# RuyiLian/CheckerPose

Hardware: NVIDIA B200
Metric: RoIs/sec (4096-kpt GNN head) (higher is better)
Workload: dtype bf16

## Files before the change

checkerpose_b200/csrc/sm100.cuh:

```cuda
#pragma once
#include <cuda_runtime.h>
#include <stdint.h>

namespace sm100 {

__device__ __forceinline__ uint32_t smem_u32(const void* p) { return (uint32_t)__cvta_generic_to_shared(p); }

__device__ __forceinline__ void mbar_init(uint64_t* bar, uint32_t count) {
  asm volatile("mbarrier.init.shared::cta.b64 [%0], %1;" ::"r"(smem_u32(bar)), "r"(count) : "memory");
}
__device__ __forceinline__ void fence_mbar_init() { asm volatile("fence.mbarrier_init.release.cluster;" ::: "memory"); }
__device__ __forceinline__ void mbar_arrive_expect_tx(uint64_t* bar, uint32_t bytes) {
  asm volatile("mbarrier.arrive.expect_tx.shared::cta.b64 _, [%0], %1;" ::"r"(smem_u32(bar)), "r"(bytes) : "memory");
}
__device__ __forceinline__ bool mbar_try_wait(uint64_t* bar, uint32_t parity) {
  uint32_t ok;
  asm volatile(
      "{\n\t.reg .pred p;\n\t"
      "mbarrier.try_wait.parity.shared::cta.b64 p, [%1], %2;\n\t"
      "selp.u32 %0, 1, 0, p;\n\t}"
      : "=r"(ok)
      : "r"(smem_u32(bar)), "r"(parity)
      : "memory");
  return ok != 0;
}
__device__ __forceinline__ void mbar_wait(uint64_t* bar, uint32_t parity) {
  if (mbar_try_wait(bar, parity)) return;
  uint32_t spins = 0;
  while (!mbar_try_wait(bar, parity)) {
    if (++spins > (1u << 27)) __trap();
  }
}

__device__ __forceinline__ bool elect_one() {
  uint32_t pred;
  asm volatile(
      "{\n\t.reg .pred p;\n\t"
      "elect.sync _|p, 0xffffffff;\n\t"
      "selp.u32 %0, 1, 0, p;\n\t}"
      : "=r"(pred));
  return pred != 0;
}

__device__ __forceinline__ void fence_proxy_async_smem() { asm volatile("fence.proxy.async.shared::cta;" ::: "memory"); }
__device__ __forceinline__ void tc_fence_before_sync() { asm volatile("tcgen05.fence::before_thread_sync;" ::: "memory"); }
__device__ __forceinline__ void tc_fence_after_sync() { asm volatile("tcgen05.fence::after_thread_sync;" ::: "memory"); }

__device__ __forceinline__ void bulk_g2s(void* smem_dst, const void* gmem_src, uint32_t bytes, uint64_t* bar) {
  asm volatile("cp.async.bulk.shared::cluster.global.mbarrier::complete_tx::bytes [%0], [%1], %2, [%3];" ::"r"(
                   smem_u32(smem_dst)),
               "l"(gmem_src), "r"(bytes), "r"(smem_u32(bar))
               : "memory");
}

__device__ __forceinline__ void tmem_alloc(uint32_t* slot_in_smem, uint32_t ncols) {
  asm volatile("tcgen05.alloc.cta_group::1.sync.aligned.shared::cta.b32 [%0], %1;" ::"r"(smem_u32(slot_in_smem)), "r"(ncols)
               : "memory");
  asm volatile("tcgen05.relinquish_alloc_permit.cta_group::1.sync.aligned;" ::: "memory");
}
__device__ __forceinline__ void tmem_dealloc(uint32_t taddr, uint32_t ncols) {
  asm volatile("tcgen05.dealloc.cta_group::1.sync.aligned.b32 %0, %1;" ::"r"(taddr), "r"(ncols) : "memory");
}

__device__ __forceinline__ void tmem_ld16(uint32_t taddr, uint32_t (&r)[16]) {
  asm volatile(
      "tcgen05.ld.sync.aligned.32x32b.x16.b32 {%0,%1,%2,%3,%4,%5,%6,%7,%8,%9,%10,%11,%12,%13,%14,%15}, [%16];"
      : "=r"(r[0]), "=r"(r[1]), "=r"(r[2]), "=r"(r[3]), "=r"(r[4]), "=r"(r[5]), "=r"(r[6]), "=r"(r[7]), "=r"(r[8]),
        "=r"(r[9]), "=r"(r[10]), "=r"(r[11]), "=r"(r[12]), "=r"(r[13]), "=r"(r[14]), "=r"(r[15])
      : "r"(taddr));
}
__device__ __forceinline__ void tmem_ld_wait() { asm volatile("tcgen05.wait::ld.sync.aligned;" ::: "memory"); }

__device__ __forceinline__ uint64_t make_smem_desc_sw128(uint32_t smem_addr) {
  return (uint64_t)((smem_addr >> 4) & 0x3FFF) | (1ull << 16) | (64ull << 32) | (1ull << 46) | (2ull << 61);
}
__device__ __forceinline__ uint32_t make_idesc_bf16_m128(uint32_t n) {
  return (1u << 4) | (1u << 7) | (1u << 10) | ((n >> 3) << 17) | ((128u >> 4) << 24);
}
__device__ __forceinline__ void mma_bf16_ss(uint32_t d_tmem, uint64_t a_desc, uint64_t b_desc, uint32_t idesc,
                                            uint32_t accumulate) {
  asm volatile(
      "{\n\t.reg .pred p;\n\t"
      "setp.ne.b32 p, %4, 0;\n\t"
      "tcgen05.mma.cta_group::1.kind::f16 [%0], %1, %2, %3, p;\n\t}"
      ::"r"(d_tmem), "l"(a_desc), "l"(b_desc), "r"(idesc), "r"(accumulate)
      : "memory");
}
__device__ __forceinline__ uint32_t smem_desc_lo(uint32_t smem_addr) { return ((smem_addr >> 4) & 0x3FFFu) | (1u << 16); }
__device__ __forceinline__ void mma_bf16_ss_lo(uint32_t d_tmem, uint32_t a_lo, uint32_t b_lo, uint32_t idesc, uint32_t accumulate) {
  asm volatile(
      "{\n\t.reg .pred p;\n\t.reg .b64 da, db;\n\t"
      "setp.ne.b32 p, %4, 0;\n\t"
      "mov.b64 da, {%1, %5};\n\t"
      "mov.b64 db, {%2, %5};\n\t"
      "tcgen05.mma.cta_group::1.kind::f16 [%0], da, db, %3, p;\n\t}"
      ::"r"(d_tmem), "r"(a_lo), "r"(b_lo), "r"(idesc), "r"(accumulate), "r"(0x40004040u)
      : "memory");
}
__device__ __forceinline__ uint32_t cluster_ctarank() {
  uint32_t r;
  asm volatile("mov.u32 %0, %%cluster_ctarank;" : "=r"(r));
  return r;
}
__device__ __forceinline__ void cluster_sync_all() {
  asm volatile("barrier.cluster.arrive.release.aligned;\n\tbarrier.cluster.wait.acquire.aligned;" ::: "memory");
}
__device__ __forceinline__ uint32_t mapa_rank(uint32_t smem_addr, uint32_t rank) {
  uint32_t r;
  asm volatile("mapa.shared::cluster.u32 %0, %1, %2;" : "=r"(r) : "r"(smem_addr), "r"(rank));
  return r;
}
__device__ __forceinline__ void mbar_arrive_cluster(uint32_t cluster_addr) {
  asm volatile("mbarrier.arrive.release.cluster.shared::cluster.b64 _, [%0];" ::"r"(cluster_addr) : "memory");
}
__device__ __forceinline__ void mbar_arrive_remote(uint32_t cluster_addr) {
  asm volatile("mbarrier.arrive.shared::cluster.b64 _, [%0];" ::"r"(cluster_addr) : "memory");
}
__device__ __forceinline__ void tmem_alloc_pair(uint32_t* slot_in_smem, uint32_t ncols) {
  asm volatile("tcgen05.alloc.cta_group::2.sync.aligned.shared::cta.b32 [%0], %1;" ::"r"(smem_u32(slot_in_smem)), "r"(ncols) : "memory");
  asm volatile("tcgen05.relinquish_alloc_permit.cta_group::2.sync.aligned;" ::: "memory");
}
__device__ __forceinline__ void tmem_dealloc_pair(uint32_t taddr, uint32_t ncols) {
  asm volatile("tcgen05.dealloc.cta_group::2.sync.aligned.b32 %0, %1;" ::"r"(taddr), "r"(ncols) : "memory");
}
__device__ __forceinline__ uint32_t make_idesc_bf16(uint32_t m, uint32_t n) {
  return (1u << 4) | (1u << 7) | (1u << 10) | ((n >> 3) << 17) | ((m >> 4) << 24);
}
__device__ __forceinline__ void mma2_bf16_ss_lo(uint32_t d_tmem, uint32_t a_lo, uint32_t b_lo, uint32_t idesc, uint32_t accumulate) {
  asm volatile(
      "{\n\t.reg .pred p;\n\t.reg .b64 da, db;\n\t"
      "setp.ne.b32 p, %4, 0;\n\t"
      "mov.b64 da, {%1, %5};\n\t"
      "mov.b64 db, {%2, %5};\n\t"
      "tcgen05.mma.cta_group::2.kind::f16 [%0], da, db, %3, p;\n\t}"
      ::"r"(d_tmem), "r"(a_lo), "r"(b_lo), "r"(idesc), "r"(accumulate), "r"(0x40004040u)
      : "memory");
}
__device__ __forceinline__ void mma2_commit_both(uint32_t bar_s) {
  asm volatile("tcgen05.commit.cta_group::2.mbarrier::arrive::one.shared::cluster.multicast::cluster.b64 [%0], %1;"
               ::"r"(bar_s), "h"((uint16_t)3) : "memory");
}

__device__ __forceinline__ void bulk_g2s_multicast(void* smem_dst, const void* gmem_src, uint32_t bytes, uint64_t* bar, uint16_t cta_mask) {
  asm volatile("cp.async.bulk.shared::cluster.global.mbarrier::complete_tx::bytes.multicast::cluster [%0], [%1], %2, [%3], %4;"
               ::"r"(smem_u32(smem_dst)), "l"(gmem_src), "r"(bytes), "r"(smem_u32(bar)), "h"(cta_mask) : "memory");
}
__device__ __forceinline__ void mma_commit_multicast(uint64_t* bar, uint16_t cta_mask) {
  asm volatile("tcgen05.commit.cta_group::1.mbarrier::arrive::one.shared::cluster.multicast::cluster.b64 [%0], %1;"
               ::"r"(smem_u32(bar)), "h"(cta_mask) : "memory");
}

__device__ __forceinline__ void mma_commit(uint64_t* bar) {
  asm volatile("tcgen05.commit.cta_group::1.mbarrier::arrive::one.shared::cluster.b64 [%0];" ::"r"(smem_u32(bar))
               : "memory");
}

}
```

checkerpose_b200/csrc/taps_chain_tcgen05.cu:

```cuda
#include <cuda.h>

#include "common.cuh"
#include "sm100.cuh"

using bf16 = __nv_bfloat16;
using namespace sm100;

namespace {

constexpr int TILE_M = 128;
constexpr int NUM_G_WARPS = 4, G_THREADS = NUM_G_WARPS * 32;
constexpr int NUM_E_WARPS = 8;
constexpr int E_WARP0 = 4;
constexpr int W_WARP = E_WARP0 + NUM_E_WARPS, MMA_WARP = W_WARP + 1;
constexpr int NUM_WARPS = 16;
static_assert(NUM_E_WARPS % 4 == 0 && E_WARP0 % 4 == 0 && NUM_G_WARPS <= E_WARP0 && TILE_M % (NUM_G_WARPS * 4) == 0, "epilogue warp w drains TMEM lane quarter w % 4");
constexpr int NTHREADS = NUM_WARPS * 32;
constexpr int CHUNK_BYTES = TILE_M * 128;
constexpr int NX = 4;
constexpr int NH = 4;
constexpr int B_STAGES = 4, B_STAGE_BYTES = 128 * 128;
constexpr int TBUF_BYTES = 32 * 64;
constexpr int BIAS_FLOATS = 1024;
constexpr int ACC_COLS = 256;
constexpr int MAX_WT = 48;

constexpr int OFF_X = 0;
constexpr int OFF_H = OFF_X + NX * CHUNK_BYTES;
constexpr int OFF_B = OFF_H + NH * CHUNK_BYTES;
constexpr int OFF_TBUF = OFF_B + B_STAGES * B_STAGE_BYTES;
constexpr int OFF_BIAS = OFF_TBUF + NUM_E_WARPS * TBUF_BYTES;
constexpr int OFF_BAR = OFF_BIAS + BIAS_FLOATS * 4;
constexpr int SMEM_BYTES = OFF_BAR + 512;
static_assert(SMEM_BYTES + 1024 <= 227 * 1024, "shared memory budget");

struct WT {
  const uint8_t* ptr;
  uint32_t bytes, pad;
};

struct TcParams {
  cp_chain_params p;
  int tiles_per_roi, num_tiles;
  int KX;
  int P2;
  int halves2;
  int T;
  WT wt[MAX_WT];
};

struct Bars {
  uint64_t x_full[NX], x_empty[NX];
  uint64_t b_full[B_STAGES], b_empty[B_STAGES];
  uint64_t h_full[NH], h_free;
  uint64_t acc_full[2], acc_empty[2];
  uint32_t tmem_slot;
};
static_assert(sizeof(Bars) <= 512, "barrier block");

__device__ __forceinline__ uint32_t chunk_off(int row, int piece) { return (uint32_t)(row * 128 + ((piece ^ (row & 7)) << 4)); }
__device__ __forceinline__ uint32_t f2_to_bf2(float lo, float hi) {
  __nv_bfloat162 v = __floats2bfloat162_rn(lo, hi);
  return *reinterpret_cast<uint32_t*>(&v);
}
__device__ __forceinline__ void mbar_arrive(uint64_t* bar) {
  asm volatile("mbarrier.arrive.shared::cta.b64 _, [%0];" ::"r"(smem_u32(bar)) : "memory");
}
__device__ __forceinline__ void cp_async16_zfill(uint32_t dst, const void* src, uint32_t src_bytes) {
  asm volatile("cp.async.cg.shared.global [%0], [%1], 16, %2;" ::"r"(dst), "l"(src), "r"(src_bytes) : "memory");
}
__device__ __forceinline__ void cp_async_arrive_noinc(uint64_t* bar) {
  asm volatile("cp.async.mbarrier.arrive.noinc.shared::cta.b64 [%0];" ::"r"(smem_u32(bar)) : "memory");
}
__device__ __forceinline__ uint4 lds128(uint32_t addr) {
  uint4 r;
  asm volatile("ld.shared.v4.u32 {%0,%1,%2,%3}, [%4];" : "=r"(r.x), "=r"(r.y), "=r"(r.z), "=r"(r.w) : "r"(addr));
  return r;
}
__device__ __forceinline__ void sts128(uint32_t addr, uint4 v) {
  asm volatile("st.shared.v4.u32 [%0], {%1,%2,%3,%4};" ::"r"(addr), "r"(v.x), "r"(v.y), "r"(v.z), "r"(v.w) : "memory");
}

__device__ void gather_warps(const TcParams& kp, uint8_t* sm, Bars* bars, int gw, int lane) {
  const cp_chain_params& p = kp.p;
  const int rg = lane >> 3, piece = lane & 7;
  const uint32_t sm_base = smem_u32(sm);
  constexpr int RPT = TILE_M / (NUM_G_WARPS * 4);
  int toff[RPT], toff_next[RPT];
  auto load_ids = [&](int tile, int (&o)[RPT]) {
    const int b = tile / kp.tiles_per_roi, n0 = (tile - b * kp.tiles_per_roi) * TILE_M;
    const int rows_valid = min(TILE_M, p.N - n0);
#pragma unroll
    for (int i = 0; i < RPT; ++i) {
      const int r = 4 * (gw + NUM_G_WARPS * i) + rg;
      o[i] = -1;
      if (r < rows_valid) {
        const size_t e = (size_t)b * p.N + n0 + r;
        const float mk = p.mask ? __ldg(p.mask + e) : 1.f;
        const int yy = (int)(2 * __ldg(p.y_id + e)), xx = (int)(2 * __ldg(p.x_id + e));
        if (yy < 0 || xx < 0 || yy + p.tap_step >= p.Hp || xx + p.tap_step >= p.Wp) __trap();
        if (mk != 0.f) o[i] = (yy * p.Wp + xx) * 128;
      }
    }
  };
  if ((int)blockIdx.x < kp.num_tiles) load_ids(blockIdx.x, toff_next);
  uint32_t cnt = 0;
  for (int tile = blockIdx.x; tile < kp.num_tiles; tile += gridDim.x) {
    const int b = tile / kp.tiles_per_roi, n0 = (tile - b * kp.tiles_per_roi) * TILE_M;
    const int rows_valid = min(TILE_M, p.N - n0);
#pragma unroll
    for (int i = 0; i < RPT; ++i) toff[i] = toff_next[i];
    if (tile + (int)gridDim.x < kp.num_tiles) load_ids(tile + gridDim.x, toff_next);
    const uint8_t* pb = reinterpret_cast<const uint8_t*>(p.patches) + (size_t)b * p.Hp * p.Wp * 128 + piece * 16;
    const uint8_t* gf = reinterpret_cast<const uint8_t*>(p.graph_feat) + ((size_t)b * p.N + n0) * p.ld_gf * 2 + piece * 16;
    for (int c = 0; c < kp.KX; ++c, ++cnt) {
      const uint32_t slot = cnt % NX;
      if (cnt >= NX) mbar_wait(&bars->x_empty[slot], ((cnt / NX) - 1) & 1);
      const uint32_t dst = sm_base + OFF_X + slot * CHUNK_BYTES;
      if (c < 4) {
        const int tap_off = (((c & 1) ? p.tap_step : 0) * p.Wp + ((c & 2) ? p.tap_step : 0)) * 128;
#pragma unroll
        for (int i = 0; i < RPT; ++i) {
          const int r = 4 * (gw + NUM_G_WARPS * i) + rg;
          const bool ok = toff[i] >= 0;
          cp_async16_zfill(dst + chunk_off(r, piece), pb + (ok ? toff[i] + tap_off : 0), ok ? 16u : 0u);
        }
      } else {
        const uint8_t* src = gf + (c - 4) * 128;
#pragma unroll
        for (int i = 0; i < RPT; ++i) {
          const int r = 4 * (gw + NUM_G_WARPS * i) + rg;
          const bool ok = r < rows_valid;
          cp_async16_zfill(dst + chunk_off(r, piece), src + (ok ? (size_t)r * p.ld_gf * 2 : 0), ok ? 16u : 0u);
        }
      }
      cp_async_arrive_noinc(&bars->x_full[slot]);
    }
  }
}

__device__ void weight_producer(const TcParams& kp, uint8_t* sm, Bars* bars) {
  uint32_t cnt = 0;
  for (int tile = blockIdx.x; tile < kp.num_tiles; tile += gridDim.x) {
    for (int w = 0; w < kp.T; ++w, ++cnt) {
      const int s = cnt % B_STAGES;
      const uint32_t use = cnt / B_STAGES;
      if (use > 0) mbar_wait(&bars->b_empty[s], (use - 1) & 1);
      if (elect_one()) {
        mbar_arrive_expect_tx(&bars->b_full[s], kp.wt[w].bytes);
        bulk_g2s(sm + OFF_B + s * B_STAGE_BYTES, kp.wt[w].ptr, kp.wt[w].bytes, &bars->b_full[s]);
      }
      __syncwarp();
    }
  }
}

__device__ void mma_issuer(const TcParams& kp, uint8_t* sm, Bars* bars, uint32_t tmem_base) {
  uint32_t wcnt = 0;
  uint32_t xcnt = 0;
  uint32_t st = 0;
  uint32_t hcnt = 0;
  const uint32_t idesc = make_idesc_bf16_m128(128);
  const uint32_t b_lo0 = smem_desc_lo(smem_u32(sm + OFF_B));
  auto gemm_block = [&](uint32_t a_addr, uint32_t d, bool accumulate) {
    const int s = wcnt % B_STAGES;
    mbar_wait(&bars->b_full[s], (wcnt / B_STAGES) & 1);
    tc_fence_after_sync();
    const uint32_t a_lo = smem_desc_lo(a_addr), b_lo = b_lo0 + s * (B_STAGE_BYTES >> 4);
    if (elect_one()) {
      mma_bf16_ss_lo(d, a_lo, b_lo, idesc, (uint32_t)accumulate);
      mma_bf16_ss_lo(d, a_lo + 2, b_lo + 2, idesc, 1u);
      mma_bf16_ss_lo(d, a_lo + 4, b_lo + 4, idesc, 1u);
      mma_bf16_ss_lo(d, a_lo + 6, b_lo + 6, idesc, 1u);
      mma_commit(&bars->b_empty[s]);
    }
    __syncwarp();
    ++wcnt;
  };
  auto acquire_acc = [&]() -> uint32_t {
    const uint32_t slot = st & 1;
    if (st >= 2) {
      mbar_wait(&bars->acc_empty[slot], ((st >> 1) - 1) & 1);
      tc_fence_after_sync();
    }
    return tmem_base + slot * ACC_COLS;
  };
  for (int tile = blockIdx.x; tile < kp.num_tiles; tile += gridDim.x) {
    {
      const uint32_t d = acquire_acc();
      for (int c = 0; c < kp.KX; ++c, ++xcnt) {
        const uint32_t slot = xcnt % NX;
        mbar_wait(&bars->x_full[slot], (xcnt / NX) & 1);
        tc_fence_after_sync();
        const uint32_t a_addr = smem_u32(sm + OFF_X + slot * CHUNK_BYTES);
        gemm_block(a_addr, d, c != 0);
        gemm_block(a_addr, d + 128, c != 0);
        if (elect_one()) mma_commit(&bars->x_empty[slot]);
        __syncwarp();
      }
      if (elect_one()) mma_commit(&bars->acc_full[st & 1]);
      __syncwarp();
      ++st;
    }
    {
      const uint32_t d = acquire_acc();
      for (int c = 0; c < NH; ++c) {
        mbar_wait(&bars->h_full[c], hcnt & 1);
        tc_fence_after_sync();
        const uint32_t a_addr = smem_u32(sm + OFF_H + c * CHUNK_BYTES);
        gemm_block(a_addr, d, c != 0);
        gemm_block(a_addr, d + 128, c != 0);
      }
      ++hcnt;
      if (elect_one()) {
        mma_commit(&bars->h_free);
        mma_commit(&bars->acc_full[st & 1]);
      }
      __syncwarp();
      ++st;
    }
    for (int half = 0; half < kp.halves2; ++half) {
      const uint32_t d = acquire_acc();
      for (int c = 0; c < NH; ++c) {
        if (half == 0) {
          mbar_wait(&bars->h_full[c], hcnt & 1);
          tc_fence_after_sync();
        }
        const uint32_t a_addr = smem_u32(sm + OFF_H + c * CHUNK_BYTES);
        for (int nb = 0; nb < kp.P2; ++nb) gemm_block(a_addr, d + nb * 128, c != 0);
      }
      if (half == 0) ++hcnt;
      if (elect_one()) {
        if (half == kp.halves2 - 1) mma_commit(&bars->h_free);
        mma_commit(&bars->acc_full[st & 1]);
      }
      __syncwarp();
      ++st;
    }
  }
}

__device__ __forceinline__ void tma_store_3d(const CUtensorMap* map, uint32_t smem_src, int c0, int c1, int c2) {
  asm volatile("cp.async.bulk.tensor.3d.global.shared::cta.bulk_group [%0, {%2, %3, %4}], [%1];"
               ::"l"(map), "r"(smem_src), "r"(c0), "r"(c1), "r"(c2) : "memory");
}
__device__ __forceinline__ void bulk_commit() { asm volatile("cp.async.bulk.commit_group;" ::: "memory"); }
__device__ __forceinline__ void bulk_wait_read0() { asm volatile("cp.async.bulk.wait_group.read 0;" ::: "memory"); }

__device__ void epilogue_warps(const TcParams& kp, const CUtensorMap* out_map, uint8_t* sm, Bars* bars, uint32_t tmem_base, int ew, int lane) {
  const cp_chain_params& p = kp.p;
  const int q = ew & 3, hh = ew >> 2;
  const int row = q * 32 + lane;
  const uint32_t sm_base = smem_u32(sm);
  const uint32_t bias_s = sm_base + OFF_BIAS;
  const uint32_t tbuf = sm_base + OFF_TBUF + ew * TBUF_BYTES;
  const int sw = (lane >> 1) & 3;
  uint32_t st = 0, hfree = 0;
  for (int tile = blockIdx.x; tile < kp.num_tiles; tile += gridDim.x) {
    const int b = tile / kp.tiles_per_roi, n0 = (tile - b * kp.tiles_per_roi) * TILE_M;
    const int rows_valid = min(TILE_M, p.N - n0);
    const int nstages = 2 + kp.halves2;
    for (int k = 0; k < nstages; ++k, ++st) {
      const uint32_t slot = st & 1;
      const int layer = k < 2 ? k : 2;
      const cp_chain_layer& L = p.layers[layer];
      const int ncols = k < 2 ? ACC_COLS : kp.P2 * 128;
      const int col0 = k < 2 ? 0 : (k - 2) * ACC_COLS;
      const uint32_t bias_l = bias_s + (uint32_t)(layer * 256 + col0) * 4;
      mbar_wait(&bars->acc_full[slot], (st >> 1) & 1);
      tc_fence_after_sync();
      if (k < 2) {
        if (hfree > 0) mbar_wait(&bars->h_free, (hfree - 1) & 1);
        ++hfree;
      }
      const uint32_t tbase = tmem_base + slot * ACC_COLS + ((uint32_t)(q * 32) << 16);
      for (int c0 = hh * 32; c0 < ncols; c0 += 32 * (NUM_E_WARPS / 4)) {
        uint32_t r[32];
        asm volatile(
            "tcgen05.ld.sync.aligned.32x32b.x32.b32 {%0,%1,%2,%3,%4,%5,%6,%7,%8,%9,%10,%11,%12,%13,%14,%15,"
            "%16,%17,%18,%19,%20,%21,%22,%23,%24,%25,%26,%27,%28,%29,%30,%31}, [%32];"
            : "=r"(r[0]), "=r"(r[1]), "=r"(r[2]), "=r"(r[3]), "=r"(r[4]), "=r"(r[5]), "=r"(r[6]), "=r"(r[7]), "=r"(r[8]),
              "=r"(r[9]), "=r"(r[10]), "=r"(r[11]), "=r"(r[12]), "=r"(r[13]), "=r"(r[14]), "=r"(r[15]), "=r"(r[16]),
              "=r"(r[17]), "=r"(r[18]), "=r"(r[19]), "=r"(r[20]), "=r"(r[21]), "=r"(r[22]), "=r"(r[23]), "=r"(r[24]),
              "=r"(r[25]), "=r"(r[26]), "=r"(r[27]), "=r"(r[28]), "=r"(r[29]), "=r"(r[30]), "=r"(r[31])
            : "r"(tbase + (uint32_t)c0));
        float v[32];
        uint4 bb[8];
#pragma unroll
        for (int e4 = 0; e4 < 8; ++e4) bb[e4] = lds128(bias_l + (uint32_t)(c0 + e4 * 4) * 4);
        tmem_ld_wait();
#pragma unroll
        for (int e4 = 0; e4 < 8; ++e4) {
          v[e4 * 4 + 0] = __uint_as_float(r[e4 * 4 + 0]) + __uint_as_float(bb[e4].x);
          v[e4 * 4 + 1] = __uint_as_float(r[e4 * 4 + 1]) + __uint_as_float(bb[e4].y);
          v[e4 * 4 + 2] = __uint_as_float(r[e4 * 4 + 2]) + __uint_as_float(bb[e4].z);
          v[e4 * 4 + 3] = __uint_as_float(r[e4 * 4 + 3]) + __uint_as_float(bb[e4].w);
        }
        if (L.act) {
#pragma unroll
          for (int e = 0; e < 32; ++e) v[e] = cp::lrelu(v[e], L.slope);
        }
        uint4 w[4];
#pragma unroll
        for (int e = 0; e < 4; ++e)
          w[e] = make_uint4(f2_to_bf2(v[e * 8], v[e * 8 + 1]), f2_to_bf2(v[e * 8 + 2], v[e * 8 + 3]),
                            f2_to_bf2(v[e * 8 + 4], v[e * 8 + 5]), f2_to_bf2(v[e * 8 + 6], v[e * 8 + 7]));
        if (k < 2) {
          const uint32_t hb = sm_base + OFF_H + (uint32_t)(c0 >> 6) * CHUNK_BYTES;
#pragma unroll
          for (int e = 0; e < 4; ++e) sts128(hb + chunk_off(row, ((c0 & 63) >> 3) + e), w[e]);
          fence_proxy_async_smem();
          __syncwarp();
          if (lane == 0) mbar_arrive(&bars->h_full[c0 >> 6]);
        } else {
          if (lane == 0) bulk_wait_read0();
          __syncwarp();
#pragma unroll
          for (int e = 0; e < 4; ++e) sts128(tbuf + lane * 64 + ((e ^ sw) << 4), w[e]);
          fence_proxy_async_smem();
          __syncwarp();
          if (lane == 0 && q * 32 < rows_valid) {
            tma_store_3d(out_map, tbuf, col0 + c0, n0 + q * 32, b);
            bulk_commit();
          }
        }
      }
      tc_fence_before_sync();
      __syncwarp();
      if (lane == 0) mbar_arrive(&bars->acc_empty[slot]);
    }
  }
  if (lane == 0) bulk_wait_read0();
}

__global__ void __launch_bounds__(NTHREADS, 1) taps_chain_kernel(const __grid_constant__ TcParams kp, const __grid_constant__ CUtensorMap out_map) {
  extern __shared__ __align__(1024) uint8_t sm[];
  if ((smem_u32(sm) & 1023u) != 0) __trap();
  Bars* bars = reinterpret_cast<Bars*>(sm + OFF_BAR);
  const int warp = threadIdx.x >> 5, lane = threadIdx.x & 31;
  if (threadIdx.x == 0) {
    for (int s = 0; s < NX; ++s) {
      mbar_init(&bars->x_full[s], G_THREADS);
      mbar_init(&bars->x_empty[s], 1);
    }
    for (int s = 0; s < B_STAGES; ++s) {
      mbar_init(&bars->b_full[s], 1);
      mbar_init(&bars->b_empty[s], 1);
    }
    for (int c = 0; c < NH; ++c) mbar_init(&bars->h_full[c], 8);
    mbar_init(&bars->h_free, 1);
    for (int s = 0; s < 2; ++s) {
      mbar_init(&bars->acc_full[s], 1);
      mbar_init(&bars->acc_empty[s], NUM_E_WARPS);
    }
    fence_mbar_init();
  }
  if (warp == W_WARP) tmem_alloc(&bars->tmem_slot, 2 * ACC_COLS);
  for (int i = threadIdx.x; i < BIAS_FLOATS; i += NTHREADS) {
    const int layer = i < 256 ? 0 : i < 512 ? 1 : 2;
    const int c = i - (layer == 2 ? 512 : layer * 256);
    const cp_chain_layer& L = kp.p.layers[layer];
    reinterpret_cast<float*>(sm + OFF_BIAS)[i] = (L.bias && c < L.nout) ? L.bias[c] : 0.f;
  }
  tc_fence_before_sync();
  __syncthreads();
  tc_fence_after_sync();
  const uint32_t tmem_base = bars->tmem_slot;

  if (warp < NUM_G_WARPS) {
    gather_warps(kp, sm, bars, warp, lane);
  } else if (warp >= E_WARP0 && warp < E_WARP0 + NUM_E_WARPS) {
    epilogue_warps(kp, &out_map, sm, bars, tmem_base, warp - E_WARP0, lane);
  } else if (warp == W_WARP) {
    weight_producer(kp, sm, bars);
  } else if (warp == MMA_WARP) {
    mma_issuer(kp, sm, bars, tmem_base);
  }
  tc_fence_before_sync();
  __syncthreads();
  if (warp == W_WARP) tmem_dealloc(tmem_base, 2 * ACC_COLS);
}

}

namespace cp {

bool taps_chain_try(const cp_chain_params& p, cudaStream_t s, int* rc) {
  *rc = CP_OK;
  if (p.prologue != CP_PRO_TAPS || p.num_layers != 3 || p.out_mode != CP_OUT_BF16 || p.a_out) return false;
  const cp_chain_layer &L0 = p.layers[0], &L1 = p.layers[1], &L2 = p.layers[2];
  if (p.E != 64 || (p.Cg != 64 && p.Cg != 128 && p.Cg != 256) || L0.kin != 256 + p.Cg || L0.nout != 256 || L1.kin != 256 ||
      L1.nout != 256 || L2.kin != 256 || (L2.nout != 256 && L2.nout != 512) || p.ld_out < L2.nout || (p.ld_out % 8) != 0 ||
      (p.ld_gf % 8) != 0 || (reinterpret_cast<uintptr_t>(p.patches) & 15) || (reinterpret_cast<uintptr_t>(p.graph_feat) & 15) ||
      (reinterpret_cast<uintptr_t>(p.out) & 15) || (size_t)p.Hp * p.Wp * 128 >= (1ull << 31))
    return false;
  TcParams kp;
  kp.p = p;
  kp.tiles_per_roi = (p.N + TILE_M - 1) / TILE_M;
  kp.num_tiles = kp.tiles_per_roi * p.B;
  kp.KX = 4 + p.Cg / 64;
  kp.halves2 = L2.nout / 256;
  kp.P2 = 2;
  int T = 0;
  auto tile_ptr = [](const cp_chain_layer& L, int nb, int kc) {
    return reinterpret_cast<const uint8_t*>(L.w_packed) + (size_t)nb * 128 * L.kin * 2 + (size_t)kc * 128 * 128;
  };
  for (int c = 0; c < kp.KX; ++c)
    for (int nb = 0; nb < 2; ++nb) kp.wt[T++] = {tile_ptr(L0, nb, c), 128 * 128, 0};
  for (int c = 0; c < NH; ++c)
    for (int nb = 0; nb < 2; ++nb) kp.wt[T++] = {tile_ptr(L1, nb, c), 128 * 128, 0};
  for (int half = 0; half < kp.halves2; ++half)
    for (int c = 0; c < NH; ++c)
      for (int nb = 0; nb < kp.P2; ++nb) kp.wt[T++] = {tile_ptr(L2, half * 2 + nb, c), 128 * 128, 0};
  kp.T = T;
  const int num_sms = cp::num_sms();
  const int grid = kp.num_tiles < num_sms ? kp.num_tiles : num_sms;
  cudaError_t e = cudaFuncSetAttribute(taps_chain_kernel, cudaFuncAttributeMaxDynamicSharedMemorySize, SMEM_BYTES);
  if (e != cudaSuccess) {
    cp::set_error("cp_chain_fwd(TAPS): cudaFuncSetAttribute failed: %s", cudaGetErrorString(e));
    *rc = CP_E_CUDA;
    return true;
  }
  CUtensorMap map;
  *rc = cp::make_out_tensor_map(&map, p.out, L2.nout, p.ld_out, p.N, p.B, "cp_chain_fwd(TAPS)");
  if (*rc != CP_OK) return true;
  taps_chain_kernel<<<grid, NTHREADS, SMEM_BYTES, s>>>(kp, map);
  e = cudaPeekAtLastError();
  if (e != cudaSuccess) {
    cp::set_error("cp_chain_fwd(TAPS): CUDA error %d (%s)", (int)e, cudaGetErrorString(e));
    (void)cudaGetLastError();
    *rc = CP_E_CUDA;
  }
  return true;
}

}
```

Measured before the change: 17610.

## Keep hidden activations in TMEM and feed later layers via TS-form MMA

```diff
diff --git a/checkerpose_b200/csrc/sm100.cuh b/checkerpose_b200/csrc/sm100.cuh
--- a/checkerpose_b200/csrc/sm100.cuh
+++ b/checkerpose_b200/csrc/sm100.cuh
@@ -70,6 +70,14 @@
       : "r"(taddr));
 }
 __device__ __forceinline__ void tmem_ld_wait() { asm volatile("tcgen05.wait::ld.sync.aligned;" ::: "memory"); }
+__device__ __forceinline__ void tmem_st16(uint32_t taddr, const uint32_t (&r)[16]) {
+  asm volatile(
+      "tcgen05.st.sync.aligned.32x32b.x16.b32 [%0], {%1,%2,%3,%4,%5,%6,%7,%8,%9,%10,%11,%12,%13,%14,%15,%16};"
+      ::"r"(taddr), "r"(r[0]), "r"(r[1]), "r"(r[2]), "r"(r[3]), "r"(r[4]), "r"(r[5]), "r"(r[6]), "r"(r[7]), "r"(r[8]),
+        "r"(r[9]), "r"(r[10]), "r"(r[11]), "r"(r[12]), "r"(r[13]), "r"(r[14]), "r"(r[15])
+      : "memory");
+}
+__device__ __forceinline__ void tmem_st_wait() { asm volatile("tcgen05.wait::st.sync.aligned;" ::: "memory"); }
 
 __device__ __forceinline__ uint64_t make_smem_desc_sw128(uint32_t smem_addr) {
   return (uint64_t)((smem_addr >> 4) & 0x3FFF) | (1ull << 16) | (64ull << 32) | (1ull << 46) | (2ull << 61);
@@ -95,6 +103,15 @@
       "mov.b64 db, {%2, %5};\n\t"
       "tcgen05.mma.cta_group::1.kind::f16 [%0], da, db, %3, p;\n\t}"
       ::"r"(d_tmem), "r"(a_lo), "r"(b_lo), "r"(idesc), "r"(accumulate), "r"(0x40004040u)
+      : "memory");
+}
+__device__ __forceinline__ void mma_bf16_ts_lo(uint32_t d_tmem, uint32_t a_tmem, uint32_t b_lo, uint32_t idesc, uint32_t accumulate) {
+  asm volatile(
+      "{\n\t.reg .pred p;\n\t.reg .b64 db;\n\t"
+      "setp.ne.b32 p, %4, 0;\n\t"
+      "mov.b64 db, {%2, %5};\n\t"
+      "tcgen05.mma.cta_group::1.kind::f16 [%0], [%1], db, %3, p;\n\t}"
+      ::"r"(d_tmem), "r"(a_tmem), "r"(b_lo), "r"(idesc), "r"(accumulate), "r"(0x40004040u)
       : "memory");
 }
 __device__ __forceinline__ uint32_t cluster_ctarank() {
diff --git a/checkerpose_b200/csrc/taps_chain_tcgen05.cu b/checkerpose_b200/csrc/taps_chain_tcgen05.cu
--- a/checkerpose_b200/csrc/taps_chain_tcgen05.cu
+++ b/checkerpose_b200/csrc/taps_chain_tcgen05.cu
@@ -14,20 +14,19 @@
 constexpr int E_WARP0 = 4;
 constexpr int W_WARP = E_WARP0 + NUM_E_WARPS, MMA_WARP = W_WARP + 1;
 constexpr int NUM_WARPS = 16;
-static_assert(NUM_E_WARPS % 4 == 0 && E_WARP0 % 4 == 0 && NUM_G_WARPS <= E_WARP0 && TILE_M % (NUM_G_WARPS * 4) == 0, "epilogue warp w drains TMEM lane quarter w % 4");
+static_assert(NUM_E_WARPS == 8 && E_WARP0 % 4 == 0 && NUM_G_WARPS <= E_WARP0 && TILE_M % (NUM_G_WARPS * 4) == 0, "epilogue warp w drains TMEM lane quarter w % 4");
 constexpr int NTHREADS = NUM_WARPS * 32;
 constexpr int CHUNK_BYTES = TILE_M * 128;
 constexpr int NX = 4;
-constexpr int NH = 4;
+constexpr int KH = 4;
 constexpr int B_STAGES = 4, B_STAGE_BYTES = 128 * 128;
 constexpr int TBUF_BYTES = 32 * 64;
 constexpr int BIAS_FLOATS = 1024;
-constexpr int ACC_COLS = 256;
+constexpr int NBLK = 4, BLK_COLS = 128;
 constexpr int MAX_WT = 48;
 
 constexpr int OFF_X = 0;
-constexpr int OFF_H = OFF_X + NX * CHUNK_BYTES;
-constexpr int OFF_B = OFF_H + NH * CHUNK_BYTES;
+constexpr int OFF_B = OFF_X + NX * CHUNK_BYTES;
 constexpr int OFF_TBUF = OFF_B + B_STAGES * B_STAGE_BYTES;
 constexpr int OFF_BIAS = OFF_TBUF + NUM_E_WARPS * TBUF_BYTES;
 constexpr int OFF_BAR = OFF_BIAS + BIAS_FLOATS * 4;
@@ -43,7 +42,6 @@
   cp_chain_params p;
   int tiles_per_roi, num_tiles;
   int KX;
-  int P2;
   int halves2;
   int T;
   WT wt[MAX_WT];
@@ -52,13 +50,23 @@
 struct Bars {
   uint64_t x_full[NX], x_empty[NX];
   uint64_t b_full[B_STAGES], b_empty[B_STAGES];
-  uint64_t h_full[NH], h_free;
-  uint64_t acc_full[2], acc_empty[2];
+  uint64_t h_ready[KH];
+  uint64_t h1_read;
+  uint64_t acc_full[NBLK], acc_empty[NBLK];
   uint32_t tmem_slot;
 };
 static_assert(sizeof(Bars) <= 512, "barrier block");
 
 __device__ __forceinline__ uint32_t chunk_off(int row, int piece) { return (uint32_t)(row * 128 + ((piece ^ (row & 7)) << 4)); }
+
+struct Roles {
+  uint32_t x, y, z, w;
+};
+__device__ __forceinline__ Roles block_roles(uint32_t it, int halves2) {
+  const uint32_t x = (it & 1) * 2, z = 2 - x;
+  return halves2 == 2 ? Roles{x, 1, z, 3} : Roles{x, x + 1, z, z + 1};
+}
+__device__ __forceinline__ uint32_t h_col(uint32_t s) { return 8u * ((s & 9u) | ((s & 2u) << 1) | ((s & 4u) >> 1)); }
 __device__ __forceinline__ uint32_t f2_to_bf2(float lo, float hi) {
   __nv_bfloat162 v = __floats2bfloat162_rn(lo, hi);
   return *reinterpret_cast<uint32_t*>(&v);
@@ -158,84 +166,103 @@
 __device__ void mma_issuer(const TcParams& kp, uint8_t* sm, Bars* bars, uint32_t tmem_base) {
   uint32_t wcnt = 0;
   uint32_t xcnt = 0;
-  uint32_t st = 0;
-  uint32_t hcnt = 0;
+  uint32_t ph = 0;
   const uint32_t idesc = make_idesc_bf16_m128(128);
   const uint32_t b_lo0 = smem_desc_lo(smem_u32(sm + OFF_B));
-  auto gemm_block = [&](uint32_t a_addr, uint32_t d, bool accumulate) {
+  auto next_weight = [&]() -> uint32_t {
     const int s = wcnt % B_STAGES;
     mbar_wait(&bars->b_full[s], (wcnt / B_STAGES) & 1);
     tc_fence_after_sync();
-    const uint32_t a_lo = smem_desc_lo(a_addr), b_lo = b_lo0 + s * (B_STAGE_BYTES >> 4);
+    return b_lo0 + s * (B_STAGE_BYTES >> 4);
+  };
+  auto gemm_ss = [&](uint32_t a_addr, uint32_t d, bool accumulate) {
+    const uint32_t b_lo = next_weight(), a_lo = smem_desc_lo(a_addr);
     if (elect_one()) {
       mma_bf16_ss_lo(d, a_lo, b_lo, idesc, (uint32_t)accumulate);
       mma_bf16_ss_lo(d, a_lo + 2, b_lo + 2, idesc, 1u);
       mma_bf16_ss_lo(d, a_lo + 4, b_lo + 4, idesc, 1u);
       mma_bf16_ss_lo(d, a_lo + 6, b_lo + 6, idesc, 1u);
-      mma_commit(&bars->b_empty[s]);
+      mma_commit(&bars->b_empty[wcnt % B_STAGES]);
     }
     __syncwarp();
     ++wcnt;
   };
-  auto acquire_acc = [&]() -> uint32_t {
-    const uint32_t slot = st & 1;
-    if (st >= 2) {
-      mbar_wait(&bars->acc_empty[slot], ((st >> 1) - 1) & 1);
-      tc_fence_after_sync();
-    }
-    return tmem_base + slot * ACC_COLS;
-  };
-  for (int tile = blockIdx.x; tile < kp.num_tiles; tile += gridDim.x) {
+  auto gemm_ts = [&](uint32_t h, int c, uint32_t d, bool accumulate) {
+    const uint32_t b_lo = next_weight();
+    if (elect_one()) {
+      mma_bf16_ts_lo(d, h + h_col(4 * c), b_lo, idesc, (uint32_t)accumulate);
+      mma_bf16_ts_lo(d, h + h_col(4 * c + 1), b_lo + 2, idesc, 1u);
+      mma_bf16_ts_lo(d, h + h_col(4 * c + 2), b_lo + 4, idesc, 1u);
+      mma_bf16_ts_lo(d, h + h_col(4 * c + 3), b_lo + 6, idesc, 1u);
+      mma_commit(&bars->b_empty[wcnt % B_STAGES]);
+    }
+    __syncwarp();
+    ++wcnt;
+  };
+  auto acquire = [&](uint32_t b) -> uint32_t {
+    mbar_wait(&bars->acc_empty[b], ((ph >> b) & 1) ^ 1);
+    tc_fence_after_sync();
+    return tmem_base + b * BLK_COLS;
+  };
+  auto filled = [&](uint32_t b) {
+    if (elect_one()) mma_commit(&bars->acc_full[b]);
+    __syncwarp();
+    ph ^= 1u << b;
+  };
+  auto wait_h = [&](int c, uint32_t parity) {
+    mbar_wait(&bars->h_ready[c], parity);
+    tc_fence_after_sync();
+  };
+  uint32_t it = 0;
+  for (int tile = blockIdx.x; tile < kp.num_tiles; tile += gridDim.x, ++it) {
+    const Roles r = block_roles(it, kp.halves2);
     {
-      const uint32_t d = acquire_acc();
+      if (it > 0) mbar_wait(&bars->h1_read, (it - 1) & 1);
+      const uint32_t d0 = acquire(r.x), d1 = acquire(r.y);
       for (int c = 0; c < kp.KX; ++c, ++xcnt) {
         const uint32_t slot = xcnt % NX;
         mbar_wait(&bars->x_full[slot], (xcnt / NX) & 1);
         tc_fence_after_sync();
         const uint32_t a_addr = smem_u32(sm + OFF_X + slot * CHUNK_BYTES);
-        gemm_block(a_addr, d, c != 0);
-        gemm_block(a_addr, d + 128, c != 0);
+        gemm_ss(a_addr, d0, c != 0);
+        gemm_ss(a_addr, d1, c != 0);
         if (elect_one()) mma_commit(&bars->x_empty[slot]);
         __syncwarp();
       }
-      if (elect_one()) mma_commit(&bars->acc_full[st & 1]);
+      filled(r.x);
+      filled(r.y);
+    }
+    {
+      const uint32_t h = tmem_base + r.x * BLK_COLS;
+      const uint32_t d0 = acquire(r.z), d1 = acquire(r.w);
+      for (int c = 0; c < KH; ++c) {
+        wait_h(c, 0);
+        gemm_ts(h, c, d0, c != 0);
+        gemm_ts(h, c, d1, c != 0);
+      }
+      filled(r.z);
+      filled(r.w);
+    }
+    {
+      const uint32_t h = tmem_base + r.z * BLK_COLS;
+      const uint32_t d0 = acquire(r.x), d1 = acquire(r.y);
+      for (int c = 0; c < KH; ++c) {
+        wait_h(c, 1);
+        gemm_ts(h, c, d0, c != 0);
+        gemm_ts(h, c, d1, c != 0);
+      }
+      filled(r.x);
+      filled(r.y);
+      if (kp.halves2 == 2) {
+        for (int nb = 0; nb < 2; ++nb) {
+          const uint32_t b = nb == 0 ? r.w : r.x;
+          const uint32_t d = acquire(b);
+          for (int c = 0; c < KH; ++c) gemm_ts(h, c, d, c != 0);
+          filled(b);
+        }
+      }
+      if (elect_one()) mma_commit(&bars->h1_read);
       __syncwarp();
-      ++st;
-    }
-    {
-      const uint32_t d = acquire_acc();
-      for (int c = 0; c < NH; ++c) {
-        mbar_wait(&bars->h_full[c], hcnt & 1);
-        tc_fence_after_sync();
-        const uint32_t a_addr = smem_u32(sm + OFF_H + c * CHUNK_BYTES);
-        gemm_block(a_addr, d, c != 0);
-        gemm_block(a_addr, d + 128, c != 0);
-      }
-      ++hcnt;
-      if (elect_one()) {
-        mma_commit(&bars->h_free);
-        mma_commit(&bars->acc_full[st & 1]);
-      }
-      __syncwarp();
-      ++st;
-    }
-    for (int half = 0; half < kp.halves2; ++half) {
-      const uint32_t d = acquire_acc();
-      for (int c = 0; c < NH; ++c) {
-        if (half == 0) {
-          mbar_wait(&bars->h_full[c], hcnt & 1);
-          tc_fence_after_sync();
-        }
-        const uint32_t a_addr = smem_u32(sm + OFF_H + c * CHUNK_BYTES);
-        for (int nb = 0; nb < kp.P2; ++nb) gemm_block(a_addr, d + nb * 128, c != 0);
-      }
-      if (half == 0) ++hcnt;
-      if (elect_one()) {
-        if (half == kp.halves2 - 1) mma_commit(&bars->h_free);
-        mma_commit(&bars->acc_full[st & 1]);
-      }
-      __syncwarp();
-      ++st;
     }
   }
 }
@@ -250,31 +277,38 @@
 __device__ void epilogue_warps(const TcParams& kp, const CUtensorMap* out_map, uint8_t* sm, Bars* bars, uint32_t tmem_base, int ew, int lane) {
   const cp_chain_params& p = kp.p;
   const int q = ew & 3, hh = ew >> 2;
-  const int row = q * 32 + lane;
   const uint32_t sm_base = smem_u32(sm);
   const uint32_t bias_s = sm_base + OFF_BIAS;
   const uint32_t tbuf = sm_base + OFF_TBUF + ew * TBUF_BYTES;
   const int sw = (lane >> 1) & 3;
-  uint32_t st = 0, hfree = 0;
-  for (int tile = blockIdx.x; tile < kp.num_tiles; tile += gridDim.x) {
+  const uint32_t tlane = tmem_base + ((uint32_t)(q * 32) << 16);
+  uint32_t ph = 0;
+  uint32_t it = 0;
+  for (int tile = blockIdx.x; tile < kp.num_tiles; tile += gridDim.x, ++it) {
     const int b = tile / kp.tiles_per_roi, n0 = (tile - b * kp.tiles_per_roi) * TILE_M;
     const int rows_valid = min(TILE_M, p.N - n0);
     const int nstages = 2 + kp.halves2;
-    for (int k = 0; k < nstages; ++k, ++st) {
-      const uint32_t slot = st & 1;
+    const Roles ro = block_roles(it, kp.halves2);
+    for (int k = 0; k < nstages; ++k) {
       const int layer = k < 2 ? k : 2;
       const cp_chain_layer& L = p.layers[layer];
-      const int ncols = k < 2 ? ACC_COLS : kp.P2 * 128;
-      const int col0 = k < 2 ? 0 : (k - 2) * ACC_COLS;
+      const int col0 = k < 2 ? 0 : (k - 2) * 256;
       const uint32_t bias_l = bias_s + (uint32_t)(layer * 256 + col0) * 4;
-      mbar_wait(&bars->acc_full[slot], (st >> 1) & 1);
-      tc_fence_after_sync();
-      if (k < 2) {
-        if (hfree > 0) mbar_wait(&bars->h_free, (hfree - 1) & 1);
-        ++hfree;
-      }
-      const uint32_t tbase = tmem_base + slot * ACC_COLS + ((uint32_t)(q * 32) << 16);
-      for (int c0 = hh * 32; c0 < ncols; c0 += 32 * (NUM_E_WARPS / 4)) {
+      const uint32_t blk0 = k == 1 ? ro.z : k == 3 ? ro.w : ro.x;
+      const uint32_t blk1 = k == 1 ? ro.w : k == 3 ? ro.x : ro.y;
+      auto release = [&](uint32_t blk) {
+        tc_fence_before_sync();
+        __syncwarp();
+        if (lane == 0) mbar_arrive(&bars->acc_empty[blk]);
+        ph ^= 1u << blk;
+      };
+      for (int i = 0; i < 4; ++i) {
+        const int c0 = i * 64 + hh * 32;
+        const uint32_t blk = i < 2 ? blk0 : blk1;
+        if ((i & 1) == 0) {
+          mbar_wait(&bars->acc_full[blk], (ph >> blk) & 1);
+          tc_fence_after_sync();
+        }
         uint32_t r[32];
         asm volatile(
             "tcgen05.ld.sync.aligned.32x32b.x32.b32 {%0,%1,%2,%3,%4,%5,%6,%7,%8,%9,%10,%11,%12,%13,%14,%15,"
@@ -283,7 +317,7 @@
               "=r"(r[9]), "=r"(r[10]), "=r"(r[11]), "=r"(r[12]), "=r"(r[13]), "=r"(r[14]), "=r"(r[15]), "=r"(r[16]),
               "=r"(r[17]), "=r"(r[18]), "=r"(r[19]), "=r"(r[20]), "=r"(r[21]), "=r"(r[22]), "=r"(r[23]), "=r"(r[24]),
               "=r"(r[25]), "=r"(r[26]), "=r"(r[27]), "=r"(r[28]), "=r"(r[29]), "=r"(r[30]), "=r"(r[31])
-            : "r"(tbase + (uint32_t)c0));
+            : "r"(tlane + blk * BLK_COLS + (uint32_t)(c0 & 127)));
         float v[32];
         uint4 bb[8];
 #pragma unroll
@@ -300,23 +334,20 @@
 #pragma unroll
           for (int e = 0; e < 32; ++e) v[e] = cp::lrelu(v[e], L.slope);
         }
-        uint4 w[4];
-#pragma unroll
-        for (int e = 0; e < 4; ++e)
-          w[e] = make_uint4(f2_to_bf2(v[e * 8], v[e * 8 + 1]), f2_to_bf2(v[e * 8 + 2], v[e * 8 + 3]),
-                            f2_to_bf2(v[e * 8 + 4], v[e * 8 + 5]), f2_to_bf2(v[e * 8 + 6], v[e * 8 + 7]));
+        uint32_t w[16];
+#pragma unroll
+        for (int e = 0; e < 16; ++e) w[e] = f2_to_bf2(v[2 * e], v[2 * e + 1]);
         if (k < 2) {
-          const uint32_t hb = sm_base + OFF_H + (uint32_t)(c0 >> 6) * CHUNK_BYTES;
-#pragma unroll
-          for (int e = 0; e < 4; ++e) sts128(hb + chunk_off(row, ((c0 & 63) >> 3) + e), w[e]);
-          fence_proxy_async_smem();
+          tmem_st16(tlane + blk0 * BLK_COLS + h_col(4 * i + 2 * hh), w);
+          tmem_st_wait();
+          tc_fence_before_sync();
           __syncwarp();
-          if (lane == 0) mbar_arrive(&bars->h_full[c0 >> 6]);
+          if (lane == 0) mbar_arrive(&bars->h_ready[i]);
         } else {
           if (lane == 0) bulk_wait_read0();
           __syncwarp();
 #pragma unroll
-          for (int e = 0; e < 4; ++e) sts128(tbuf + lane * 64 + ((e ^ sw) << 4), w[e]);
+          for (int e = 0; e < 4; ++e) sts128(tbuf + lane * 64 + ((e ^ sw) << 4), make_uint4(w[4 * e], w[4 * e + 1], w[4 * e + 2], w[4 * e + 3]));
           fence_proxy_async_smem();
           __syncwarp();
           if (lane == 0 && q * 32 < rows_valid) {
@@ -324,10 +355,12 @@
             bulk_commit();
           }
         }
-      }
-      tc_fence_before_sync();
-      __syncwarp();
-      if (lane == 0) mbar_arrive(&bars->acc_empty[slot]);
+        if (i == 1 && k >= 2) release(blk0);
+        if (i == 3) {
+          if (k < 2) release(blk0);
+          release(blk1);
+        }
+      }
     }
   }
   if (lane == 0) bulk_wait_read0();
@@ -347,15 +380,15 @@
       mbar_init(&bars->b_full[s], 1);
       mbar_init(&bars->b_empty[s], 1);
     }
-    for (int c = 0; c < NH; ++c) mbar_init(&bars->h_full[c], 8);
-    mbar_init(&bars->h_free, 1);
-    for (int s = 0; s < 2; ++s) {
+    for (int c = 0; c < KH; ++c) mbar_init(&bars->h_ready[c], 8);
+    mbar_init(&bars->h1_read, 1);
+    for (int s = 0; s < NBLK; ++s) {
       mbar_init(&bars->acc_full[s], 1);
       mbar_init(&bars->acc_empty[s], NUM_E_WARPS);
     }
     fence_mbar_init();
   }
-  if (warp == W_WARP) tmem_alloc(&bars->tmem_slot, 2 * ACC_COLS);
+  if (warp == W_WARP) tmem_alloc(&bars->tmem_slot, NBLK * BLK_COLS);
   for (int i = threadIdx.x; i < BIAS_FLOATS; i += NTHREADS) {
     const int layer = i < 256 ? 0 : i < 512 ? 1 : 2;
     const int c = i - (layer == 2 ? 512 : layer * 256);
@@ -378,7 +411,7 @@
   }
   tc_fence_before_sync();
   __syncthreads();
-  if (warp == W_WARP) tmem_dealloc(tmem_base, 2 * ACC_COLS);
+  if (warp == W_WARP) tmem_dealloc(tmem_base, NBLK * BLK_COLS);
 }
 
 }
@@ -400,18 +433,19 @@
   kp.num_tiles = kp.tiles_per_roi * p.B;
   kp.KX = 4 + p.Cg / 64;
   kp.halves2 = L2.nout / 256;
-  kp.P2 = 2;
   int T = 0;
   auto tile_ptr = [](const cp_chain_layer& L, int nb, int kc) {
     return reinterpret_cast<const uint8_t*>(L.w_packed) + (size_t)nb * 128 * L.kin * 2 + (size_t)kc * 128 * 128;
   };
   for (int c = 0; c < kp.KX; ++c)
     for (int nb = 0; nb < 2; ++nb) kp.wt[T++] = {tile_ptr(L0, nb, c), 128 * 128, 0};
-  for (int c = 0; c < NH; ++c)
+  for (int c = 0; c < KH; ++c)
     for (int nb = 0; nb < 2; ++nb) kp.wt[T++] = {tile_ptr(L1, nb, c), 128 * 128, 0};
-  for (int half = 0; half < kp.halves2; ++half)
-    for (int c = 0; c < NH; ++c)
-      for (int nb = 0; nb < kp.P2; ++nb) kp.wt[T++] = {tile_ptr(L2, half * 2 + nb, c), 128 * 128, 0};
+  for (int c = 0; c < KH; ++c)
+    for (int nb = 0; nb < 2; ++nb) kp.wt[T++] = {tile_ptr(L2, nb, c), 128 * 128, 0};
+  if (kp.halves2 == 2)
+    for (int nb = 2; nb < 4; ++nb)
+      for (int c = 0; c < KH; ++c) kp.wt[T++] = {tile_ptr(L2, nb, c), 128 * 128, 0};
   kp.T = T;
   const int num_sms = cp::num_sms();
   const int grid = kp.num_tiles < num_sms ? kp.num_tiles : num_sms;
```

After: 17700 (median of 6 runs). No clear change (+0.5%).
